# hrz2000/CustomNeRF

Hardware: AMD Instinct MI355X
Metric: training rays/s (higher is better)
Workload: dtype f16

## Files before the change

customnerf_amd/csrc/gridencoder_binned.hip:

```cpp
#include "grid_common.h"
#include "optim_common.h"
#include <vector>
#include <algorithm>
#include <cstdio>

#define BN_CHUNK_LOG2 12
#define BN_CHUNK (1u << BN_CHUNK_LOG2)
#define BN_THREADS 256
#define BN_PPT 4
#define BN_PTS (BN_THREADS * BN_PPT)
#define BN_MAX_CHUNKS 512
#define BN_SEG (1u << 18)

struct BinPlan {
    uint32_t bin_first[GE_MAX_LEVELS + 1];
    uint32_t nb;
    uint32_t total_bins;
};

struct BinWs {
    uint32_t *hist;
    uint32_t *bin_base;
    uint32_t *seg_first;
    void *records;
// ... 123 lines not shown
        }
        __syncthreads();
        if (tid == 0) { carry_r = cr + tr; carry_s = cs + ts; }
        __syncthreads();
    }
    if (tid == 0) {
        bin_base[total_bins] = carry_r; seg_first[total_bins] = carry_s;
        if (split_list) split_list[0] = n_split;
    }
}

template <typename T>
__global__ void __launch_bounds__(BN_THREADS) k_bin_emit(const T *__restrict__ grad, const float *__restrict__ inputs, const GridLevels lv,
                                                         const BinPlan plan, const uint32_t *__restrict__ hist,
                                                         const uint32_t *__restrict__ bin_base, BinRec<T> *__restrict__ records, uint32_t B,
                                                         uint32_t gridtype, int align_corners, uint32_t interp, float *__restrict__ grad_grid,
                                                         float *__restrict__ found_inf) {
    __shared__ uint32_t cursor[BN_MAX_CHUNKS];
    const uint32_t level = blockIdx.x / plan.nb, pb = blockIdx.x % plan.nb;
    const uint32_t nch = plan.bin_first[level + 1] - plan.bin_first[level];
    for (uint32_t c = threadIdx.x; c < nch; c += BN_THREADS) {
        const uint32_t bin = plan.bin_first[level] + c;
        cursor[c] = bin_base[bin] + hist[(size_t)bin * plan.nb + pb];
    }
    __syncthreads();
#pragma unroll
    for (int i = 0; i < BN_PPT; i++) {
        const uint32_t b = pb * BN_PTS + i * BN_THREADS + threadIdx.x;
        float in[3];
        if (!bn_load_point(inputs, b, B, in)) continue;
        uint32_t index[8];
        float wgt[8];
        bn_corners(in, lv, level, gridtype, align_corners, interp, index, wgt);
        using Vec = FeatVec<T, 2>;
        const Vec g = reinterpret_cast<const Vec *>(grad)[(size_t)level * B + b];
        const float g0 = ge_to_float(g.v[0]), g1 = ge_to_float(g.v[1]);
        if constexpr (sizeof(T) == 2) {
            if (!(fabsf(g0) <= 65504.0f) || !(fabsf(g1) <= 65504.0f)) {
                grad_grid[((size_t)lv.offset[level] + index[0]) * 2] = __builtin_nanf("");
                if (found_inf) *found_inf = 1.0f;
            }
        } else {
            if ((!(fabsf(g0) <= 3.4e38f) || !(fabsf(g1) <= 3.4e38f)) && found_inf) *found_inf = 1.0f;
        }
        struct alignas(8) RecPair { BinRec<T> a, b; };
#pragma unroll
        for (int q = 0; q < 4; q++) {
            const uint32_t i0 = index[2 * q], i1 = index[2 * q + 1];
            const uint32_t c0 = i0 >> BN_CHUNK_LOG2, c1 = i1 >> BN_CHUNK_LOG2;
            RecPair rp;
            rp.a.idx = i0 & (BN_CHUNK - 1);
            rp.b.idx = i1 & (BN_CHUNK - 1);
            if constexpr (sizeof(T) == 2) {
                rp.a.v = __floats2half2_rn(wgt[2 * q] * g0, wgt[2 * q] * g1);
                rp.b.v = __floats2half2_rn(wgt[2 * q + 1] * g0, wgt[2 * q + 1] * g1);
            } else {
                rp.a.v0 = wgt[2 * q] * g0; rp.a.v1 = wgt[2 * q] * g1;
                rp.b.v0 = wgt[2 * q + 1] * g0; rp.b.v1 = wgt[2 * q + 1] * g1;
            }
            const uint32_t pos0 = atomicAdd(&cursor[c0], c0 == c1 ? 2u : 1u);
            if (c0 == c1) {
                *reinterpret_cast<RecPair *>(records + pos0) = rp;
            } else {
                const uint32_t pos1 = atomicAdd(&cursor[c1], 1u);
                records[pos0] = rp.a;
                records[pos1] = rp.b;
            }
        }
    }
}

#define BN_FIX_BITS 24
template <typename T> struct BinAcc;
template <> struct BinAcc<__half> { using type = long long; };
template <> struct BinAcc<float> { using type = float; };

template <typename T>
__device__ __forceinline__ void bn_add_record(typename BinAcc<T>::type *acc, const BinRec<T> &r) {
    if constexpr (sizeof(T) == 2) {
        const float2 f = __half22float2(r.v);
        const long long a = (long long)(f.x * 16777216.0f), b = (long long)(f.y * 16777216.0f);
        atomicAdd(reinterpret_cast<unsigned long long *>(&acc[r.idx * 2]), (unsigned long long)a);
        atomicAdd(reinterpret_cast<unsigned long long *>(&acc[r.idx * 2 + 1]), (unsigned long long)b);
    } else {
        unsafeAtomicAdd(&acc[r.idx * 2], r.v0);
        unsafeAtomicAdd(&acc[r.idx * 2 + 1], r.v1);
    }
}

template <typename T>
__device__ __forceinline__ float bn_acc_to_float(typename BinAcc<T>::type a) {
    if constexpr (sizeof(T) == 2) return (float)((double)a * (1.0 / 16777216.0));
    else return a;
}

template <typename T>
__global__ void __launch_bounds__(1024) k_bin_accum(const BinRec<T> *__restrict__ records, const uint32_t *__restrict__ bin_base,
                                                    const uint32_t *__restrict__ seg_first, const GridLevels lv, const BinPlan plan,
                                                    float *__restrict__ grad_grid) {
    using A = typename BinAcc<T>::type;
    extern __shared__ __attribute__((aligned(16))) unsigned char bn_lds[];
    A *acc = reinterpret_cast<A *>(bn_lds);
    uint32_t &s_bin = *reinterpret_cast<uint32_t *>(bn_lds + sizeof(A) * BN_CHUNK * 2);
    const uint32_t nseg_total = seg_first[plan.total_bins];
    if (blockIdx.x >= nseg_total) return;
    if (threadIdx.x == 0) {
        uint32_t lo = 0, hi = plan.total_bins;
        while (lo < hi) {
            const uint32_t mid = (lo + hi) >> 1;
            if (seg_first[mid + 1] <= blockIdx.x) lo = mid + 1; else hi = mid;
        }
        s_bin = lo;
    }
    for (uint32_t i = threadIdx.x; i < sizeof(A) * BN_CHUNK * 2 / 16; i += 1024) reinterpret_cast<uint4 *>(bn_lds)[i] = make_uint4(0, 0, 0, 0);
    __syncthreads();
    const uint32_t bin = s_bin;
    const uint32_t seg = blockIdx.x - seg_first[bin], nseg = seg_first[bin + 1] - seg_first[bin];
    const uint32_t r0 = bin_base[bin], r1 = bin_base[bin + 1];
    const uint32_t begin = r0 + seg * BN_SEG, end = min(begin + BN_SEG, r1);
    constexpr int UNR = 4;
    uint32_t i = begin + threadIdx.x;
    for (; i + (UNR - 1) * 1024 < end; i += UNR * 1024) {
        BinRec<T> r[UNR];
#pragma unroll
        for (int u = 0; u < UNR; u++) r[u] = records[i + u * 1024];
#pragma unroll
        for (int u = 0; u < UNR; u++) bn_add_record<T>(acc, r[u]);
    }
    for (; i < end; i += 1024) bn_add_record<T>(acc, records[i]);
    __syncthreads();
    uint32_t level = 0;
    while (plan.bin_first[level + 1] <= bin) level++;
    const uint32_t chunk = bin - plan.bin_first[level];
    const uint32_t e0 = chunk << BN_CHUNK_LOG2;
    const uint32_t n_entries = min(BN_CHUNK, lv.size[level] - e0);
    float *__restrict__ dst = grad_grid + ((size_t)lv.offset[level] + e0) * 2;
    if (nseg == 1) {
        for (uint32_t j = threadIdx.x; j < n_entries * 2 / 4; j += 1024) {
            float4 g = reinterpret_cast<float4 *>(dst)[j];
            g.x += bn_acc_to_float<T>(acc[j * 4]); g.y += bn_acc_to_float<T>(acc[j * 4 + 1]);
            g.z += bn_acc_to_float<T>(acc[j * 4 + 2]); g.w += bn_acc_to_float<T>(acc[j * 4 + 3]);
            reinterpret_cast<float4 *>(dst)[j] = g;
        }
    } else {
        for (uint32_t j = threadIdx.x; j < n_entries * 2; j += 1024) {
            const float a = bn_acc_to_float<T>(acc[j]);
            if (a != 0.0f) unsafeAtomicAdd(&dst[j], a);
        }
    }
}


#define B3_SINGLE 15u


__device__ __forceinline__ void b3_pairs(const float (&in)[3], const GridLevels &lv, uint32_t level, uint32_t gridtype, bool align_corners,
                                         uint32_t interp, uint32_t (&i0)[4], uint32_t (&i1)[4], float (&wyz)[4], float &fx) {
    const uint32_t hashmap_size = lv.size[level];
    const float scale = lv.scale[level];
    const uint32_t resolution = lv.resolution[level];
    float pos[3];
    uint32_t pos_grid[3];
#pragma unroll
    for (int d = 0; d < 3; d++) {
        pos[d] = cn_fma(in[d], scale, align_corners ? 0.0f : 0.5f);
        pos_grid[d] = (uint32_t)floorf(pos[d]);
        pos[d] -= (float)pos_grid[d];
        if (interp == 1) pos[d] = ge_smoothstep(pos[d]);
    }
    fx = pos[0];
    const float oy = 1 - pos[1], oz = 1 - pos[2];
    wyz[0] = oy * oz; wyz[1] = pos[1] * oz; wyz[2] = oy * pos[2]; wyz[3] = pos[1] * pos[2];
    const int mode = ge_level_mode<3>(gridtype, align_corners, hashmap_size, resolution);
    if (mode == GE_MODE_HASH2) {
        const uint32_t mask = hashmap_size - 1;
        const uint32_t hy0 = pos_grid[1] * 2654435761u, hy1 = hy0 + 2654435761u, hz0 = pos_grid[2] * 805459861u, hz1 = hz0 + 805459861u;
        const uint32_t hyz[4] = {hy0 ^ hz0, hy1 ^ hz0, hy0 ^ hz1, hy1 ^ hz1};
        const uint32_t x0 = pos_grid[0], x1 = x0 + 1;
#pragma unroll
        for (int q = 0; q < 4; q++) { i0[q] = (x0 ^ hyz[q]) & mask; i1[q] = (x1 ^ hyz[q]) & mask; }
    } else if (mode == GE_MODE_DENSE) {
        const uint32_t s1 = align_corners ? resolution : resolution + 1, s2 = s1 * s1;
        const uint32_t lin = pos_grid[0] + pos_grid[1] * s1 + pos_grid[2] * s2;
        i0[0] = lin; i0[1] = lin + s1; i0[2] = lin + s2; i0[3] = lin + s1 + s2;
#pragma unroll
        for (int q = 0; q < 4; q++) i1[q] = i0[q] + 1;
        if (align_corners) {
#pragma unroll
            for (int q = 0; q < 4; q++) {
                if (i0[q] >= hashmap_size) i0[q] -= hashmap_size;
                if (i1[q] >= hashmap_size) i1[q] -= hashmap_size;
            }
        }
    } else {
        ge_dispatch_mode(mode, [&](auto mode_c) {
#pragma unroll
        for (int q = 0; q < 4; q++) {
            uint32_t pgl[3] = {pos_grid[0], pos_grid[1] + (q & 1), pos_grid[2] + (q >> 1)};
            i0[q] = ge_index_m<3, decltype(mode_c)::value>(gridtype, align_corners, hashmap_size, resolution, pgl);
            pgl[0] += 1;
            i1[q] = ge_index_m<3, decltype(mode_c)::value>(gridtype, align_corners, hashmap_size, resolution, pgl);
        }
        });
    }
}

__device__ __forceinline__ bool b3_paired_d(uint32_t i0, uint32_t i1) {
    const uint32_t m = i0 ^ i1;
    return m != 0 && (m >> BN_CHUNK_LOG2) == 0 && (m & (m + 1)) == 0;
}

__device__ __forceinline__ uint32_t b3_ticket(uint32_t *counters, uint32_t c) {
    const uint64_t act = __ballot(1);
    const uint32_t c_lead = __builtin_amdgcn_readfirstlane(c);
    if (__ballot(c == c_lead) == act) {
        const uint32_t rank = __builtin_amdgcn_mbcnt_hi((uint32_t)(act >> 32), __builtin_amdgcn_mbcnt_lo((uint32_t)act, 0u));
        uint32_t base = 0;
        if (rank == 0) base = atomicAdd(&counters[c_lead], (uint32_t)__popcll(act));
        return __builtin_amdgcn_readfirstlane(base) + rank;
    }
    return atomicAdd(&counters[c], 1u);
}

__device__ __forceinline__ void b3_poison(float g0, float g1, float *__restrict__ grad_grid, const GridLevels &lv, uint32_t level, uint32_t entry,
                                          float *__restrict__ found_inf) {
    if (!(fabsf(g0) <= 65504.0f) || !(fabsf(g1) <= 65504.0f)) {
        grad_grid[((size_t)lv.offset[level] + entry) * 2] = __builtin_nanf("");
        if (found_inf) *found_inf = 1.0f;
    }
}

__device__ __forceinline__ unsigned long long b3_fix(float a) {
    const double y = (double)a + 6755399441055744.0;
    return __builtin_bit_cast(unsigned long long, y) - 0x4338000000000000ull;
}
__device__ __forceinline__ void b3_add(long long *acc, uint32_t e, float a, float b) {
    atomicAdd(reinterpret_cast<unsigned long long *>(&acc[e]), b3_fix(a));
    atomicAdd(reinterpret_cast<unsigned long long *>(&acc[BN_CHUNK + e]), b3_fix(b));
}

__device__ __forceinline__ void b3_add_record(long long *acc, const uint2 r) {
    union { uint32_t u; __half2 h; } v;
    v.u = r.y;
    const float2 f = __half22float2(v.h);
    const uint32_t e = r.x & (BN_CHUNK - 1), t = (r.x >> 12) & 15u;
    if (t == B3_SINGLE) {
        b3_add(acc, e, f.x * 16777216.0f, f.y * 16777216.0f);
    } else {
        const float w1 = (float)(r.x >> 16) * (1.0f / 65536.0f), w0 = 1.0f - w1;
        const float w1s = w1 * 16777216.0f, w0s = w0 * 16777216.0f;
        b3_add(acc, e, w0s * f.x, w0s * f.y);
        b3_add(acc, e ^ ((2u << t) - 1u), w1s * f.x, w1s * f.y);
    }
}

#ifndef B3_WALK
#define B3_WALK 8
#endif
struct B3Pending { uint32_t key; unsigned long long a0, b0, a1, b1; };
__device__ __forceinline__ void b3_flush_pending(long long *acc, const B3Pending &c) {
    if (c.key == 0xFFFFFFFFu) return;
    const uint32_t e = c.key & (BN_CHUNK - 1), t = (c.key >> 12) & 15u;
    atomicAdd(reinterpret_cast<unsigned long long *>(&acc[e]), c.a0);
    atomicAdd(reinterpret_cast<unsigned long long *>(&acc[BN_CHUNK + e]), c.b0);
    if (t != B3_SINGLE) {
        const uint32_t e1 = e ^ ((2u << t) - 1u);
        atomicAdd(reinterpret_cast<unsigned long long *>(&acc[e1]), c.a1);
        atomicAdd(reinterpret_cast<unsigned long long *>(&acc[BN_CHUNK + e1]), c.b1);
    }
}
__device__ __forceinline__ void b3_push_record(long long *acc, B3Pending &c, const uint2 r) {
    union { uint32_t u; __half2 h; } v;
    v.u = r.y;
    const float2 f = __half22float2(v.h);
    const uint32_t key = r.x & 0xFFFFu, t = (r.x >> 12) & 15u;
    unsigned long long a0, b0, a1 = 0, b1 = 0;
    if (t == B3_SINGLE) {
        a0 = b3_fix(f.x * 16777216.0f); b0 = b3_fix(f.y * 16777216.0f);
    } else {
        const float w1 = (float)(r.x >> 16) * (1.0f / 65536.0f), w0 = 1.0f - w1;
        const float w1s = w1 * 16777216.0f, w0s = w0 * 16777216.0f;
        a0 = b3_fix(w0s * f.x); b0 = b3_fix(w0s * f.y);
        a1 = b3_fix(w1s * f.x); b1 = b3_fix(w1s * f.y);
    }
    if (key == c.key) {
        c.a0 += a0; c.b0 += b0; c.a1 += a1; c.b1 += b1;
    } else {
        b3_flush_pending(acc, c);
        c.key = key; c.a0 = a0; c.b0 = b0; c.a1 = a1; c.b1 = b1;
    }
}

#ifndef B3_PTS
#define B3_PTS 2048
#endif
#ifndef B3_THREADS
#define B3_THREADS 1024
#endif
#define B3_CAP (B3_PTS * 4 + 640)
#define B3_NARROW_CHUNKS 128
#define B3_WIDE_CHUNKS BN_MAX_CHUNKS
#ifndef B3_WALK_BLOCKS
#define B3_WALK_BLOCKS 256
#endif
#define B3_MAXT (B3_WALK_BLOCKS + 8)
#define B3_REGION (B3_PTS * 8)

struct Bin3Slots {
    uint32_t bin_first[GE_MAX_LEVELS + 1];
    uint32_t nb;
    uint32_t total_bins;
};

struct Bin3Plan {
    Bin3Slots p;
    uint32_t capb;
    uint32_t dense_slot[GE_MAX_LEVELS];
    uint8_t hbits[GE_MAX_LEVELS];
};

#ifndef B3_K
#define B3_K 7u
#endif
__device__ __forceinline__ uint32_t b3_bin_of(uint32_t e, uint32_t hbits) { return (e >> B3_K) & ((1u << hbits) - 1u); }
__device__ __forceinline__ uint32_t b3_local_of(uint32_t e, uint32_t hbits) { return ((e >> (B3_K + hbits)) << B3_K) | (e & ((1u << B3_K) - 1u)); }
__device__ __forceinline__ uint32_t b3_entry_of(uint32_t local, uint32_t bin, uint32_t hbits) {
    return ((local >> B3_K) << (B3_K + hbits)) | (bin << B3_K) | (local & ((1u << B3_K) - 1u));
}
__device__ __forceinline__ bool b3_paired_h(uint32_t i0, uint32_t i1) {
    const uint32_t m = i0 ^ i1;
    return m != 0 && m < (1u << B3_K) && (m & (m + 1)) == 0;
}

__global__ void __launch_bounds__(B3_THREADS, B3_THREADS >= 1024 ? 8 : 4) k_bin3_emit(const __half *__restrict__ grad, const float *__restrict__ inputs, const GridLevels lv,
                                                          const Bin3Plan plan, uint32_t *__restrict__ runs, uint32_t *__restrict__ cursor,
                                                          uint2 *__restrict__ hslab, uint2 *__restrict__ dslab, uint32_t B,
                                                          uint32_t gridtype, int align_corners, uint32_t interp, float *__restrict__ grad_grid, uint32_t n_slots,
                                                          uint32_t abl_arg, float *__restrict__ found_inf) {
#ifdef CNERF_TUNING
    const uint32_t abl = abl_arg;
#else
    constexpr uint32_t abl = 0;
    (void)abl_arg;
#endif
    extern __shared__ __attribute__((aligned(16))) unsigned char b3_lds[];
    uint2 *s_rec = reinterpret_cast<uint2 *>(b3_lds);
    uint8_t *s_bin = b3_lds + (size_t)B3_CAP * 8;
    const uint32_t nb = plan.p.nb;
    const uint32_t slot = blockIdx.x % n_slots, pb = blockIdx.x / n_slots;
    const uint32_t level = lv.order[slot];
    const uint32_t bin0 = plan.p.bin_first[slot], nch = plan.p.bin_first[slot + 1] - bin0;
    const bool dense_lvl = plan.dense_slot[slot] != 0xFFFFFFFFu;
    const uint32_t hb = plan.hbits[slot];
    const bool wide = nch > B3_NARROW_CHUNKS;
    const uint32_t NBN = wide ? B3_WIDE_CHUNKS : B3_NARROW_CHUNKS;
    uint32_t *cnt = reinterpret_cast<uint32_t *>(b3_lds + (size_t)B3_CAP * (wide ? 8 : 9));
    uint32_t *start = cnt + NBN;
    uint32_t *gdst = start + NBN;
    uint32_t *s_total = gdst + NBN;
    auto bin_of = [&](uint32_t e) { return dense_lvl ? e >> BN_CHUNK_LOG2 : b3_bin_of(e, hb); };
    auto local_of = [&](uint32_t e) { return dense_lvl ? e & (BN_CHUNK - 1) : b3_local_of(e, hb); };
    auto paired = [&](uint32_t a, uint32_t b) { return dense_lvl ? b3_paired_d(a, b) : b3_paired_h(a, b); };
    if (threadIdx.x < NBN) cnt[threadIdx.x] = 0;
    __syncthreads();
    constexpr int PPT = B3_PTS / B3_THREADS;
    bool ok[PPT];
    uint32_t i0[PPT][4], i1[PPT][4], tk[PPT][4];
    float wyz[PPT][4], fx[PPT], g0[PPT], g1[PPT];
    float in_[PPT][3];
    FeatVec<__half, 2> gh[PPT];
#pragma unroll
    for (int i = 0; i < PPT; i++) {
        const uint32_t bc = min(pb * B3_PTS + i * B3_THREADS + threadIdx.x, B - 1);
        ge_load_coords<3>(inputs, bc, in_[i]);
        gh[i] = reinterpret_cast<const FeatVec<__half, 2> *>(grad)[(size_t)level * B + bc];
    }
#pragma unroll
    for (int i = 0; i < PPT; i++) {
        const uint32_t b = pb * B3_PTS + i * B3_THREADS + threadIdx.x;
        const float (&in)[3] = in_[i];
        ok[i] = b < B && !(in[0] < 0 || in[0] > 1 || in[1] < 0 || in[1] > 1 || in[2] < 0 || in[2] > 1);
        g0[i] = __half2float(gh[i].v[0]); g1[i] = __half2float(gh[i].v[1]);
        ok[i] = ok[i] && (g0[i] != 0.0f || g1[i] != 0.0f);
        fx[i] = 0.0f;
        if (ok[i]) {
            if (abl & 32) {
#pragma unroll
                for (int q = 0; q < 4; q++) { i0[i][q] = (b * 4 + q) * 2654435761u % lv.size[level]; i1[i][q] = i0[i][q] ^ 1u; wyz[i][q] = 0.25f; }
                fx[i] = in[0] - floorf(in[0]);
            } else {
                b3_pairs(in, lv, level, gridtype, align_corners, interp, i0[i], i1[i], wyz[i], fx[i]);
            }
            b3_poison(g0[i], g1[i], grad_grid, lv, level, i0[i][0], found_inf);
#pragma unroll
            for (int q = 0; q < 4; q++) {
                if (abl & 16) { tk[i][q] = 0; continue; }
                const uint32_t c0 = bin_of(i0[i][q]);
                if (paired(i0[i][q], i1[i][q])) {
                    tk[i][q] = dense_lvl ? b3_ticket(cnt, c0) : atomicAdd(&cnt[c0], 1u);
                } else {
                    const uint32_t t0 = atomicAdd(&cnt[c0], 1u);
                    const uint32_t t1 = atomicAdd(&cnt[bin_of(i1[i][q])], 1u);
                    tk[i][q] = t0 | (t1 << 16);
                }
            }
        }
    }
    __syncthreads();
    uint32_t res_a = 0, res_b = 0;
    if (wide) {
        if (threadIdx.x < 64) {
            const uint32_t lane = threadIdx.x;
            constexpr uint32_t KPL = B3_WIDE_CHUNKS / 64;
            uint32_t c8[KPL], loc = 0;
#pragma unroll
            for (uint32_t k = 0; k < KPL; k++) { c8[k] = cnt[lane * KPL + k]; loc += c8[k]; }
            const uint32_t incl = cn_wave_incl_scan(loc);
            uint32_t run = incl - loc;
#pragma unroll
            for (uint32_t k = 0; k < KPL; k++) {
                const uint32_t c = lane * KPL + k;
                start[c] = run;
                if (dense_lvl && c < nch && !(abl & 8)) runs[(size_t)(bin0 + c) * nb + pb] = c8[k] | (run << 16);
                run += c8[k];
            }
            if (lane == 63) *s_total = incl;
        }
        asm volatile("s_waitcnt lgkmcnt(0)" ::: "memory");
        __builtin_amdgcn_s_barrier();
        asm volatile("" ::: "memory");
        if (!dense_lvl && !(abl & 1) && threadIdx.x <= NBN / 2) {
            const uint32_t b_lo = ((bin0 >> 1) + threadIdx.x) * 2u;
            uint32_t sa[2] = {0u, 0u};
#pragma unroll
            for (int h = 0; h < 2; h++) {
                const uint32_t c = b_lo + h - bin0;
                if (c < nch) {
                    const uint32_t n = cnt[c], st0 = start[c];
                    sa[h] = st0 >= B3_CAP ? 0u : min(n, (uint32_t)B3_CAP - st0);
                }
            }
            if (sa[0] | sa[1]) {
                const unsigned long long old = atomicAdd(reinterpret_cast<unsigned long long *>(cursor + b_lo), (unsigned long long)sa[0] | ((unsigned long long)sa[1] << 32));
                res_a = (uint32_t)old & 0x7FFFFFFFu;
                res_b = (uint32_t)(old >> 32) & 0x7FFFFFFFu;
            }
        }
    } else if (threadIdx.x < 64) {
        const uint32_t lane = threadIdx.x;
        const uint32_t ca = cnt[2 * lane], cb = cnt[2 * lane + 1];
        const uint32_t incl = cn_wave_incl_scan(ca + cb);
        const uint32_t oa = incl - (ca + cb), ob = oa + ca;
        start[2 * lane] = oa; start[2 * lane + 1] = ob;
        if (lane == 63) *s_total = incl;
        if (dense_lvl) {
            if (2 * lane < nch && !(abl & 8)) runs[(size_t)(bin0 + 2 * lane) * nb + pb] = ca | (oa << 16);
            if (2 * lane + 1 < nch && !(abl & 8)) runs[(size_t)(bin0 + 2 * lane + 1) * nb + pb] = cb | (ob << 16);
        } else if (!(abl & 1)) {
            const uint32_t sa = (2 * lane < nch && oa < B3_CAP) ? min(ca, (uint32_t)B3_CAP - oa) : 0u;
            const uint32_t sb = (2 * lane + 1 < nch && ob < B3_CAP) ? min(cb, (uint32_t)B3_CAP - ob) : 0u;
            if ((bin0 & 1u) == 0) {
                if (sa | sb) {
                    const unsigned long long old = atomicAdd(reinterpret_cast<unsigned long long *>(cursor + bin0 + 2 * lane),
                                                             (unsigned long long)sa | ((unsigned long long)sb << 32));
                    res_a = (uint32_t)old & 0x7FFFFFFFu;
                    res_b = (uint32_t)(old >> 32) & 0x7FFFFFFFu;
                }
            } else {
                if (sa) res_a = atomicAdd(&cursor[bin0 + 2 * lane], sa) & 0x7FFFFFFFu;
                if (sb) res_b = atomicAdd(&cursor[bin0 + 2 * lane + 1], sb) & 0x7FFFFFFFu;
            }
        }
    }
    asm volatile("s_waitcnt lgkmcnt(0)" ::: "memory");
    __builtin_amdgcn_s_barrier();
    asm volatile("" ::: "memory");
    uint2 *__restrict__ region = dslab + ((size_t)slot * nb + pb) * B3_REGION;
#pragma unroll
    for (int i = 0; i < PPT; i++) {
        if (!ok[i] || (abl & 4)) continue;
        const uint32_t fxq = min((uint32_t)(fx[i] * 65536.0f), 65535u);
        union { __half2 h; uint32_t u; } v;
        auto put = [&](uint32_t c, uint32_t ticket, uint32_t word, uint32_t val) {
            const uint32_t sl = start[c] + ticket;
            if (sl < B3_CAP) { s_rec[sl] = make_uint2(word, val); if (!wide) s_bin[sl] = (uint8_t)c; }
            else region[sl] = make_uint2(word, val);
        };
#pragma unroll
        for (int q = 0; q < 4; q++) {
            const uint32_t a0 = i0[i][q], a1 = i1[i][q];
            const uint32_t c0 = bin_of(a0);
            if (paired(a0, a1)) {
                const uint32_t t = 31u - (uint32_t)__clz((int)(a0 ^ a1));
                v.h = __floats2half2_rn(wyz[i][q] * g0[i], wyz[i][q] * g1[i]);
                put(c0, tk[i][q], local_of(a0) | (t << 12) | (fxq << 16), v.u);
            } else {
                const float w0 = (1 - fx[i]) * wyz[i][q], w1 = fx[i] * wyz[i][q];
                v.h = __floats2half2_rn(w0 * g0[i], w0 * g1[i]);
                put(c0, tk[i][q] & 0xFFFFu, local_of(a0) | (B3_SINGLE << 12), v.u);
                v.h = __floats2half2_rn(w1 * g0[i], w1 * g1[i]);
                put(bin_of(a1), tk[i][q] >> 16, local_of(a1) | (B3_SINGLE << 12), v.u);
            }
        }
    }
    if (!dense_lvl && wide) {
        if (threadIdx.x <= NBN / 2) {
            const uint32_t capb = plan.capb, b_lo = ((bin0 >> 1) + threadIdx.x) * 2u;
#pragma unroll
            for (int h = 0; h < 2; h++) {
                const uint32_t c = b_lo + h - bin0;
                if (c >= nch) continue;
                const uint32_t n = cnt[c], st0 = start[c], res = h ? res_b : res_a;
                const uint32_t staged = st0 >= B3_CAP ? 0u : min(n, (uint32_t)B3_CAP - st0);
                const uint32_t room = res >= capb ? 0u : capb - res;
                const uint32_t fit = min(min(n, room), staged);
                gdst[c] = res - st0;
                cnt[c] = fit;
                if (!(abl & 8)) runs[(size_t)(bin0 + c) * nb + pb] = (n - fit) | ((st0 + fit) << 16);
                if (n > fit) atomicOr(&cursor[bin0 + c], 0x80000000u);
            }
        }
    } else if (!dense_lvl && threadIdx.x < 64) {
        const uint32_t capb = plan.capb;
#pragma unroll
        for (int h = 0; h < 2; h++) {
            const uint32_t c = 2 * threadIdx.x + h;
            const uint32_t n = cnt[c], st0 = start[c], res = h ? res_b : res_a;
            const uint32_t staged = st0 >= B3_CAP ? 0u : min(n, (uint32_t)B3_CAP - st0);
            const uint32_t room = res >= capb ? 0u : capb - res;
            const uint32_t fit = min(min(n, room), staged);
            gdst[c] = res - st0;
            cnt[c] = fit;
            if (c < nch && !(abl & 8)) runs[(size_t)(bin0 + c) * nb + pb] = (n - fit) | ((st0 + fit) << 16);
            if (c < nch && n > fit) atomicOr(&cursor[bin0 + c], 0x80000000u);
        }
    }
    __syncthreads();
    const uint32_t total = (abl & 2) ? 0u : min(*s_total, (uint32_t)B3_CAP);
    if (dense_lvl) {
        for (uint32_t sl = threadIdx.x; sl < total; sl += B3_THREADS) region[sl] = s_rec[sl];
    } else if (wide) {
        const uint32_t capb = plan.capb, l16 = threadIdx.x & 15, grp = threadIdx.x >> 4;
        for (uint32_t c = grp; c < nch; c += B3_THREADS / 16) {
            const uint32_t st0 = start[c], en = min(c + 1 < NBN ? start[c + 1] : *s_total, total), fit = cnt[c], gd = gdst[c];
            for (uint32_t sl = st0 + l16; sl < en; sl += 16) {
                if (sl - st0 < fit) hslab[(size_t)(bin0 + c) * capb + (gd + sl)] = s_rec[sl];
                else region[sl] = s_rec[sl];
            }
        }
    } else {
        const uint32_t capb = plan.capb;
        for (uint32_t sl = threadIdx.x; sl < total; sl += B3_THREADS) {
            const uint32_t c = s_bin[sl];
            const uint32_t pos = gdst[c] + sl;
            if (sl - start[c] < cnt[c]) hslab[(size_t)(bin0 + c) * capb + pos] = s_rec[sl];
            else region[sl] = s_rec[sl];
        }
    }
}

__global__ void __launch_bounds__(BN_SCAN_THREADS) k_bin3_totals(const uint32_t *__restrict__ runs, uint32_t *__restrict__ pre, const uint32_t *__restrict__ cursor,
                                                                 uint32_t *__restrict__ bin_total, const Bin3Plan plan, uint32_t n_slots) {
    constexpr uint32_t NW = BN_SCAN_THREADS / 64;
    __shared__ uint32_t wave_tot[NW];
    __shared__ uint32_t carry;
    const uint32_t bin = blockIdx.x, nb = plan.p.nb;
    uint32_t slot = 0;
    while (slot + 1 < n_slots && plan.p.bin_first[slot + 1] <= bin) slot++;
    const bool hashed = plan.dense_slot[slot] == 0xFFFFFFFFu;
    if (hashed) {
        const uint32_t cw = cursor[bin], c = cw & 0x7FFFFFFFu;
        if (!(cw >> 31)) {
            if (threadIdx.x == 0) bin_total[bin] = min(c, plan.capb);
            return;
        }
    }
    const uint32_t *h = runs + (size_t)bin * nb;
    uint32_t *o = pre + (size_t)bin * nb;
    const uint32_t tid = threadIdx.x, lane = tid & 63, wave = tid >> 6;
    if (tid == 0) carry = 0;
    __syncthreads();
    for (uint32_t s0 = 0; s0 < nb; s0 += BN_SCAN_THREADS * 4) {
        const uint32_t i = s0 + tid * 4;
        uint32_t v[4];
#pragma unroll
        for (int k = 0; k < 4; k++) v[k] = i + k < nb ? (h[i + k] & 0xFFFFu) : 0;
        const uint32_t mine = v[0] + v[1] + v[2] + v[3];
        const uint32_t incl = cn_wave_incl_scan(mine);
        if (lane == 63) wave_tot[wave] = incl;
        __syncthreads();
        uint32_t wbase = 0, tot = 0;
#pragma unroll
        for (uint32_t w = 0; w < NW; w++) {
            const uint32_t t = wave_tot[w];
            if (w < wave) wbase += t;
            tot += t;
        }
        const uint32_t base = carry;
        uint32_t run = base + wbase + incl - mine;
#pragma unroll
        for (int k = 0; k < 4; k++) {
            if (i + k < nb) o[i + k] = run;
            run += v[k];
        }
        __syncthreads();
        if (tid == 0) carry = base + tot;
        __syncthreads();
    }
    if (tid == 0) bin_total[bin] = hashed ? min(cursor[bin] & 0x7FFFFFFFu, plan.capb) + carry : carry;
}

struct B3Adam {
    float *p, *m, *v;
    __half *ph;
    const float *state;
    float lr, beta1, beta2, eps, extra_inv;
    int zero_grad, on;
    const float *cst;
};
struct B3AdamConst { float gscale, step_size, rsqrt_bc2; int skip; };
__device__ __forceinline__ B3AdamConst b3_adam_const(const B3Adam &ad) {
    B3AdamConst c;
    c.gscale = ad.cst[0]; c.step_size = ad.cst[1]; c.rsqrt_bc2 = ad.cst[2]; c.skip = ad.cst[3] != 0.0f;
    return c;
}
__device__ __forceinline__ void b3_adam_update(const B3Adam &ad, const B3AdamConst &c, size_t idx, float4 gg, float4 pp, float4 mm, float4 vv, float4 *d4) {
    const CnAdamK ak = {c.gscale, c.step_size, c.rsqrt_bc2, ad.beta1, ad.beta2, ad.eps};
    float *pa = &pp.x, *ga = &gg.x, *ma = &mm.x, *va = &vv.x;
#pragma unroll
    for (int k = 0; k < 4; k++) cn_adam_elem(pa[k], ma[k], va[k], ga[k], ak);
    *reinterpret_cast<float4 *>(ad.p + idx) = pp;
    *reinterpret_cast<float4 *>(ad.m + idx) = mm;
    *reinterpret_cast<float4 *>(ad.v + idx) = vv;
    *d4 = ad.zero_grad ? make_float4(0, 0, 0, 0) : gg;
    if (ad.ph) *reinterpret_cast<uint2 *>(ad.ph + idx) = cn_pack_half4(pp);
}
__device__ __forceinline__ void b3_adam_apply(const B3Adam &ad, const B3AdamConst &c, size_t idx, float4 gg, float4 *d4) {
    if (c.skip) {
        *d4 = ad.zero_grad ? make_float4(0, 0, 0, 0) : gg;
        return;
    }
    b3_adam_update(ad, c, idx, gg, *reinterpret_cast<const float4 *>(ad.p + idx), *reinterpret_cast<const float4 *>(ad.m + idx),
                   *reinterpret_cast<const float4 *>(ad.v + idx), d4);
}

__device__ __forceinline__ void b3_flush(const long long *acc, const GridLevels &lv, const Bin3Slots &plan, uint32_t slot, uint32_t bin, uint32_t nseg, uint32_t gseg,
                                         float *__restrict__ grad_grid, long long *__restrict__ partial, uint32_t hbits, const B3Adam &ad,
                                         const B3AdamConst &adc) {
    const uint32_t level = lv.order[slot];
    const uint32_t cb = bin - plan.bin_first[slot];
    const uint32_t e0 = hbits == 0xFFu ? cb << BN_CHUNK_LOG2 : 0u;
    const uint32_t n_entries = hbits == 0xFFu ? min(BN_CHUNK, lv.size[level] - e0) : min(BN_CHUNK, lv.size[level] >> hbits);
    float *__restrict__ dst = grad_grid + (size_t)lv.offset[level] * 2;
    if (nseg == 1 && ad.on && !adc.skip) {
        constexpr int NIT = BN_CHUNK / 2 / 1024;
        float4 gg[NIT], pp[NIT], mm[NIT], vv[NIT];
        auto index_of = [&](uint32_t j) {
            const uint32_t e = hbits == 0xFFu ? e0 + 2 * j : b3_entry_of(2 * j, cb, hbits);
            return ((size_t)lv.offset[level] + e) * 2;
        };
#pragma unroll
        for (int it = 0; it < NIT; it++) {
            const uint32_t j = it * 1024 + threadIdx.x;
            if (j < n_entries / 2) {
                const size_t idx = index_of(j);
                gg[it] = *reinterpret_cast<const float4 *>(grad_grid + idx);
                pp[it] = *reinterpret_cast<const float4 *>(ad.p + idx);
                mm[it] = *reinterpret_cast<const float4 *>(ad.m + idx);
                vv[it] = *reinterpret_cast<const float4 *>(ad.v + idx);
            }
        }
#pragma unroll
        for (int it = 0; it < NIT; it++) {
            const uint32_t j = it * 1024 + threadIdx.x;
            if (j >= n_entries / 2) continue;
            const size_t idx = index_of(j);
            float4 g = gg[it];
            g.x += bn_acc_to_float<__half>(acc[j * 2]); g.y += bn_acc_to_float<__half>(acc[BN_CHUNK + j * 2]);
            g.z += bn_acc_to_float<__half>(acc[j * 2 + 1]); g.w += bn_acc_to_float<__half>(acc[BN_CHUNK + j * 2 + 1]);
            b3_adam_update(ad, adc, idx, g, pp[it], mm[it], vv[it], reinterpret_cast<float4 *>(grad_grid + idx));
        }
    } else if (nseg == 1) {
        for (uint32_t j = threadIdx.x; j < n_entries / 2; j += 1024) {
            const uint32_t e = hbits == 0xFFu ? e0 + 2 * j : b3_entry_of(2 * j, cb, hbits);
            float4 *d4 = reinterpret_cast<float4 *>(dst + (size_t)e * 2);
            float4 g = *d4;
            g.x += bn_acc_to_float<__half>(acc[j * 2]); g.y += bn_acc_to_float<__half>(acc[BN_CHUNK + j * 2]);
            g.z += bn_acc_to_float<__half>(acc[j * 2 + 1]); g.w += bn_acc_to_float<__half>(acc[BN_CHUNK + j * 2 + 1]);
            if (ad.on) b3_adam_apply(ad, adc, ((size_t)lv.offset[level] + e) * 2, g, d4);
            else *d4 = g;
        }
    } else {
        long long *__restrict__ img = partial + (size_t)gseg * (BN_CHUNK * 2);
        for (uint32_t j = threadIdx.x; j < n_entries * 2; j += 1024) img[j] = acc[(j & 1) * BN_CHUNK + (j >> 1)];
    }
}

#define B3_RS_GROUPS 64
#ifndef B3_RS_BINS
#define B3_RS_BINS 256
#endif
__global__ void __launch_bounds__(256) k_bin3_reduce_split(const long long *__restrict__ partial, const uint32_t *__restrict__ seg_first,
                                                           const GridLevels lv, const Bin3Plan plan, float *__restrict__ grad_grid, uint32_t n_slots,
                                                           const uint32_t *__restrict__ split_list, const B3Adam ad) {
    __shared__ long long s_sum[3][B3_RS_GROUPS][4];
    const uint32_t n_split = split_list ? split_list[0] : gridDim.x;
    if (blockIdx.x >= n_split) return;
    B3AdamConst adc = {0.0f, 0.0f, 0.0f, 0};
    if (ad.on) adc = b3_adam_const(ad);
    for (uint32_t b = blockIdx.x; b < n_split; b += gridDim.x) {
    const uint32_t bin = split_list ? split_list[1 + b] : b;
// ... 247 lines not shown
    return (uint32_t)((s + k - 1) / k);
}

static uint32_t b3_max_bins(const Bin3Slots &plan, uint32_t nl) {
    uint32_t m = 1;
    for (uint32_t s = 0; s < nl; s++) m = m > plan.bin_first[s + 1] - plan.bin_first[s] ? m : plan.bin_first[s + 1] - plan.bin_first[s];
    return m;
}

struct Bin3Ws {
    uint32_t *runs, *pre, *cursor, *bin_base, *seg_first, *seg_bin, *split_list;
    float *adam_const;
    uint2 *hslab, *dslab;
    long long *partial;
    uint64_t max_seg, cursor_bytes;
};

static bool b3_is_dense(const GridLevels &lv, uint32_t level, int ac) {
    const uint64_t r1 = (uint64_t)lv.resolution[level] + (ac ? 0 : 1);
    return r1 * r1 * r1 <= lv.size[level];
}

static bool b3_plan(const GridLevels &lv, uint32_t nl, uint32_t B, Bin3Plan &plan, uint32_t &n_dense, int ac) {
    Bin3Slots &ps = plan.p;
    ps.nb = cn_div_up(B, B3_PTS);
    uint32_t acc = 0;
    for (uint32_t s = 0; s < nl; s++) {
        ps.bin_first[s] = acc;
        acc += cn_div_up(lv.size[lv.order[s]], BN_CHUNK);
    }
    for (uint32_t s = nl; s <= GE_MAX_LEVELS; s++) ps.bin_first[s] = acc;
    ps.total_bins = acc;
    n_dense = 0;
    uint64_t cap = 0;
    bool ok = true;
    for (uint32_t s = 0; s < GE_MAX_LEVELS; s++) { plan.dense_slot[s] = 0xFFFFFFFFu; plan.hbits[s] = 0; }
    for (uint32_t s = 0; s < nl; s++) {
        const uint32_t level = lv.order[s], size = lv.size[level];
        if (b3_is_dense(lv, level, ac)) { plan.dense_slot[s] = n_dense++; continue; }
        const uint32_t nch = ps.bin_first[s + 1] - ps.bin_first[s];
        if ((size & (size - 1)) != 0 || (nch & (nch - 1)) != 0 || !(size == nch * BN_CHUNK || (nch == 1 && size >= 32))) ok = false;
        uint32_t hb = 0;
        while ((1u << hb) < nch) hb++;
        plan.hbits[s] = (uint8_t)hb;
        const uint64_t mean = (uint64_t)B * 17 / 4 / nch;
        const uint64_t c = mean + mean / 2 + 8192;
        cap = cap > c ? cap : c;
    }
    plan.capb = (uint32_t)((cap + 1) & ~(uint64_t)1);
    return ok;
}

static bool b3_enabled(const GridLevels &lv, uint32_t nl, uint32_t B, int dtype, uint32_t gridtype, int ac) {
    static const int on = cn_tune_env("CNERF_B3", 1);
    static const int wide_on = cn_tune_env("CNERF_B3_WIDE", 1);
    (void)gridtype;
    if (!on || dtype != CNERF_F16) return false;
    Bin3Plan plan;
    uint32_t nd;
    if (!b3_plan(lv, nl, B, plan, nd, ac)) return false;
    const uint32_t mc = b3_max_bins(plan.p, nl);
    if (mc > (wide_on ? (uint32_t)B3_WIDE_CHUNKS : (uint32_t)B3_NARROW_CHUNKS)) return false;
    if ((uint64_t)plan.p.total_bins * plan.capb >= 0xF0000000ull) return false;
    return (uint64_t)nl * plan.p.nb * B3_REGION < 0xF0000000ull && (uint64_t)B * 8 < 0x7FFFFFFFull;
}

static uint64_t b3_layout(const Bin3Plan &plan, uint32_t n_dense, uint32_t B, uint32_t nl, Bin3Ws *ws, void *base) {
    const Bin3Slots &ps = plan.p;
    uint64_t off = 0;
    const uint64_t o_runs = off; off = bn_align(off + (uint64_t)ps.total_bins * ps.nb * 4);
    const uint64_t o_pre = off; off = bn_align(off + (uint64_t)ps.total_bins * ps.nb * 4);
    const uint64_t o_cur = off; off = bn_align(off + ((uint64_t)ps.total_bins + 2) * 4);
    const uint64_t o_base = off; off = bn_align(off + (uint64_t)(ps.total_bins + 1) * 4);
    const uint64_t o_seg = off; off = bn_align(off + (uint64_t)(ps.total_bins + 1) * 4);
    const uint64_t o_split = off; off = bn_align(off + (uint64_t)(ps.total_bins + 1) * 4);
    const uint64_t o_adamc = off; off = bn_align(off + 16);
    const uint64_t h_records = (uint64_t)ps.total_bins * plan.capb;
    const uint64_t d_records = (uint64_t)nl * ps.nb * B3_REGION;
    (void)n_dense;
    const uint64_t o_h = off; off = bn_align(off + h_records * 8);
    const uint64_t o_d = off; off = bn_align(off + d_records * 8);
    const uint64_t max_seg = (uint64_t)ps.total_bins + cn_div_up64((uint64_t)B * nl * 8, b3_seg(B, b3_max_bins(ps, nl)));
    const uint64_t o_segbin = off; off = bn_align(off + max_seg * 4);
    const uint64_t o_part = off; off = bn_align(off + max_seg * BN_CHUNK * 2 * 8);
    if (ws) {
        char *p = (char *)base;
        ws->runs = (uint32_t *)(p + o_runs);
        ws->pre = (uint32_t *)(p + o_pre);
        ws->cursor = (uint32_t *)(p + o_cur);
        ws->cursor_bytes = (uint64_t)ps.total_bins * 4;
        ws->bin_base = (uint32_t *)(p + o_base);
        ws->seg_first = (uint32_t *)(p + o_seg);
        ws->split_list = (uint32_t *)(p + o_split);
        ws->adam_const = (float *)(p + o_adamc);
        ws->hslab = (uint2 *)(p + o_h);
        ws->dslab = (uint2 *)(p + o_d);
        ws->seg_bin = (uint32_t *)(p + o_segbin);
        ws->partial = (long long *)(p + o_part);
        ws->max_seg = max_seg;
    }
    return off;
}

__global__ void __launch_bounds__(256) k_bin3_zero(uint32_t *__restrict__ p, uint32_t n) {
    const uint32_t i = blockIdx.x * 256 + threadIdx.x;
    if (i < n) p[i] = 0;
}

static CnerfGridAdam g_grid_adam;
static bool g_grid_adam_armed = false;
static int g_grid_adam_consumed = 0;
void bn_grid_adam_arm(const CnerfGridAdam *cfg) {
    g_grid_adam_armed = cfg != nullptr;
    if (cfg) { g_grid_adam = *cfg; g_grid_adam_consumed = 0; }
}
int bn_grid_adam_consumed() { const int c = g_grid_adam_consumed; g_grid_adam_consumed = 0; return c; }
static B3Adam b3_take_adam(float *gemb, const GridLevels &lv, uint32_t nl, bool third_form) {
    B3Adam ad = {};
    if (!g_grid_adam_armed || g_grid_adam.g != gemb) return ad;
    g_grid_adam_armed = false;
    const uint64_t covered = ((uint64_t)lv.offset[nl - 1] + lv.size[nl - 1]) * 2;
    if (!third_form || covered != g_grid_adam.n) return ad;
    ad.p = g_grid_adam.p; ad.m = g_grid_adam.m; ad.v = g_grid_adam.v; ad.ph = reinterpret_cast<__half *>(g_grid_adam.p_half);
    ad.state = g_grid_adam.scaler_state;
    ad.lr = g_grid_adam.lr; ad.beta1 = g_grid_adam.beta1; ad.beta2 = g_grid_adam.beta2; ad.eps = g_grid_adam.eps; ad.extra_inv = g_grid_adam.extra_inv;
    ad.zero_grad = g_grid_adam.zero_grad; ad.on = 1;
    g_grid_adam_consumed = 1;
    return ad;
}

static int b3_backward(const __half *grad, const float *inputs, const GridLevels &lv, float *gemb, uint32_t B, uint32_t nl, uint32_t gridtype, int ac,
                       uint32_t interp, void *workspace, hipStream_t st) {
    if (nl == 0) return CNERF_OK;
    Bin3Plan plan;
    uint32_t n_dense;
    if (!b3_plan(lv, nl, B, plan, n_dense, ac)) return CNERF_EINVAL;
    Bin3Ws ws;
    b3_layout(plan, n_dense, B, nl, &ws, workspace);
    static const int emit_pad = cn_tune_env("CNERF_B3_EMIT_LDS_PAD", 0);
    const uint32_t lds_n = B3_CAP * 9 + B3_NARROW_CHUNKS * 12 + 16, lds_w = B3_CAP * 8 + B3_WIDE_CHUNKS * 12 + 16;
    const uint32_t emit_lds = (lds_n > lds_w ? lds_n : lds_w) + (uint32_t)emit_pad, acc_lds = BN_CHUNK * 2 * sizeof(long long) + 32 + B3_MAXT * 8;
    static bool attr_set = false;
    if (!attr_set) {
        (void)hipFuncSetAttribute(reinterpret_cast<const void *>(&k_bin3_emit), hipFuncAttributeMaxDynamicSharedMemorySize, emit_lds);
        (void)hipFuncSetAttribute(reinterpret_cast<const void *>(&k_bin3_accum), hipFuncAttributeMaxDynamicSharedMemorySize, acc_lds);
        attr_set = true;
    }
    const Bin3Slots &ps = plan.p;
    const uint32_t seg = b3_seg(B, b3_max_bins(ps, nl));
    B3Adam ad = b3_take_adam(gemb, lv, nl, true);
    ad.cst = ws.adam_const;
    hipLaunchKernelGGL(k_bin3_zero, dim3(cn_div_up(ps.total_bins, 256)), dim3(256), 0, st, ws.cursor, ps.total_bins);
    cn_stage(0, st);
    hipLaunchKernelGGL(k_bin3_emit, dim3(ps.nb * nl), dim3(B3_THREADS), emit_lds, st, grad, inputs, lv, plan, ws.runs, ws.cursor, ws.hslab, ws.dslab, B, gridtype, ac,
                       interp, gemb, nl, (uint32_t)cn_tune_env("CNERF_B3_EMIT_ABL", 0), g_cn_found_inf);
    cn_stage(1, st);
    hipLaunchKernelGGL(k_bin3_totals, dim3(ps.total_bins), dim3(BN_SCAN_THREADS), 0, st, (const uint32_t *)ws.runs, ws.pre, (const uint32_t *)ws.cursor, ws.bin_base,
                       plan, nl);
    static const uint32_t rs_bins = (uint32_t)cn_tune_env("CNERF_B3_RS_BINS", B3_RS_BINS);
    static const int rs_list = cn_tune_env("CNERF_B3_RSLIST", 1);
    hipLaunchKernelGGL(k_bin_scan_bins, dim3(1), dim3(1024), 0, st, ws.bin_base, ws.bin_base, ws.seg_first, ps.total_bins, seg, ws.seg_bin, ws.split_list, ad.on,
                       ad.state, ad.lr, ad.beta1, ad.beta2, ad.extra_inv, ad.on ? ws.adam_const : (float *)nullptr);
    hipLaunchKernelGGL(k_bin3_accum, dim3((uint32_t)ws.max_seg), dim3(1024), acc_lds, st, (const uint2 *)ws.hslab, (const uint2 *)ws.dslab, (const uint32_t *)ws.runs,
                       (const uint32_t *)ws.pre, (const uint32_t *)ws.cursor, (const uint32_t *)ws.bin_base, (const uint32_t *)ws.seg_first, lv, plan, gemb, ws.partial,
                       (const uint32_t *)ws.seg_bin, nl, seg, (uint32_t)cn_tune_env("CNERF_B3_ONLY", 0), ad);
    cn_stage(2, st);
    hipLaunchKernelGGL(k_bin3_reduce_split, dim3(!rs_list || ps.total_bins < rs_bins ? ps.total_bins : rs_bins, BN_CHUNK * 2 / 4 / B3_RS_GROUPS), dim3(256), 0, st,
                       (const long long *)ws.partial, ws.seg_first, lv, plan, gemb, nl, rs_list ? (const uint32_t *)ws.split_list : (const uint32_t *)nullptr, ad);
    cn_stage(3, st);
#ifdef CNERF_TUNING
    static const int dbg = cn_tune_env("CNERF_B3_DEBUG", 0);
    static int dbg_calls = 0;
    if (dbg && (++dbg_calls % dbg) == 0) {
        uint32_t n_split = 0, n_seg = 0;
        (void)hipStreamSynchronize(st);
        (void)hipMemcpy(&n_split, ws.split_list, 4, hipMemcpyDeviceToHost);
        (void)hipMemcpy(&n_seg, ws.seg_first + ps.total_bins, 4, hipMemcpyDeviceToHost);
        std::vector<uint32_t> sf(ps.total_bins + 1), bb(ps.total_bins + 1);
        (void)hipMemcpy(sf.data(), ws.seg_first, sf.size() * 4, hipMemcpyDeviceToHost);
        (void)hipMemcpy(bb.data(), ws.bin_base, bb.size() * 4, hipMemcpyDeviceToHost);
        fprintf(stderr, "[b3] call %d: bins %u segments %u split bins %u seg %u | per slot (bins, segments, records, max bin):", dbg_calls, ps.total_bins, n_seg, n_split, seg);
        for (uint32_t sl = 0; sl < nl; sl++) {
            uint32_t mx = 0;
            for (uint32_t b_ = ps.bin_first[sl]; b_ < ps.bin_first[sl + 1]; b_++) mx = std::max(mx, bb[b_ + 1] - bb[b_]);
            fprintf(stderr, " L%u(%u,%u,%u,%u)", lv.order[sl], ps.bin_first[sl + 1] - ps.bin_first[sl], sf[ps.bin_first[sl + 1]] - sf[ps.bin_first[sl]],
                    bb[ps.bin_first[sl + 1]] - bb[ps.bin_first[sl]], mx);
        }
        fprintf(stderr, "\n");
    }
#endif
    return cn_launch_status();
}

bool bn_eligible(uint32_t B, uint32_t D, uint32_t C, uint32_t nl, const GridLevels &lv) {
    if (D != 3 || C != 2 || nl == 0) return false;
    for (uint32_t l = 0; l < nl; l++)
        if (cn_div_up(lv.size[l], BN_CHUNK) > BN_MAX_CHUNKS || (lv.size[l] & 7)) return false;
    return (uint64_t)B * nl * 8 < 0xF0000000ull;
}

uint64_t bn_workspace_bytes(uint32_t B, uint32_t nl, const GridLevels &lv, int dtype) {
    uint64_t b3 = 0;
    for (int ac = 0; ac < 2; ac++) {
        if (!b3_enabled(lv, nl, B, dtype, 0u, ac)) continue;
        Bin3Plan p3;
        uint32_t nd;
        b3_plan(lv, nl, B, p3, nd, ac);
        const uint64_t b = b3_layout(p3, nd, B, nl, nullptr, nullptr);
        b3 = b > b3 ? b : b3;
    }
    BinPlan plan;
    bn_plan(lv, nl, B, plan);
    const uint64_t b1 = bn_layout(plan, B, nl, dtype, nullptr, nullptr);
    return b1 > b3 ? b1 : b3;
}

static int bn_prepare(const float *inputs, const GridLevels &lv, uint32_t B, uint32_t nl, uint32_t gridtype, int ac, uint32_t interp, int dtype,
               void *workspace, hipStream_t st) {
    BinPlan plan;
    bn_plan(lv, nl, B, plan);
    BinWs ws;
    bn_layout(plan, B, nl, dtype, &ws, workspace);
    const dim3 grid1(plan.nb * nl);
    hipLaunchKernelGGL(k_bin_hist, grid1, dim3(BN_THREADS), 0, st, inputs, lv, plan, ws.hist, B, gridtype, ac, interp);
    hipLaunchKernelGGL(k_bin_scan_blocks, dim3(plan.total_bins), dim3(BN_SCAN_THREADS), 0, st, ws.hist, ws.bin_base, plan.nb);
    hipLaunchKernelGGL(k_bin_scan_bins, dim3(1), dim3(1024), 0, st, ws.bin_base, ws.bin_base, ws.seg_first, plan.total_bins, BN_SEG, (uint32_t *)nullptr);
    return cn_launch_status();
}

template <typename T>
static int bn_phase2(const T *grad, const float *inputs, const GridLevels &lv, float *gemb, uint32_t B, uint32_t nl, uint32_t gridtype, int ac,
                     uint32_t interp, int dtype, void *workspace, hipStream_t st) {
    BinPlan plan;
    bn_plan(lv, nl, B, plan);
    BinWs ws;
    bn_layout(plan, B, nl, dtype, &ws, workspace);
    const dim3 grid1(plan.nb * nl);
    hipLaunchKernelGGL((k_bin_emit<T>), grid1, dim3(BN_THREADS), 0, st, grad, inputs, lv, plan, ws.hist, ws.bin_base, (BinRec<T> *)ws.records, B,
                       gridtype, ac, interp, gemb, g_cn_found_inf);
    const uint64_t max_seg = (uint64_t)plan.total_bins + cn_div_up64((uint64_t)B * nl * 8, BN_SEG);
    const uint32_t lds_bytes = BN_CHUNK * 2 * sizeof(typename BinAcc<T>::type) + 16;
    static bool attr_set = false;
    if (!attr_set) {
        (void)hipFuncSetAttribute(reinterpret_cast<const void *>(&k_bin_accum<T>), hipFuncAttributeMaxDynamicSharedMemorySize, lds_bytes);
        attr_set = true;
    }
    hipLaunchKernelGGL((k_bin_accum<T>), dim3((uint32_t)max_seg), dim3(1024), lds_bytes, st, (const BinRec<T> *)ws.records,
                       ws.bin_base, ws.seg_first, lv, plan, gemb);
    return cn_launch_status();
}

int bn_backward(const void *grad, const float *inputs, const GridLevels &lv, float *gemb, uint32_t B, uint32_t nl, uint32_t gridtype, int ac,
                uint32_t interp, int dtype, void *workspace, hipStream_t st) {
    if (b3_enabled(lv, nl, B, dtype, gridtype, ac)) return b3_backward((const __half *)grad, inputs, lv, gemb, B, nl, gridtype, ac, interp, workspace, st);
    if (nl) (void)b3_take_adam(gemb, lv, nl, false);
    const int rc = bn_prepare(inputs, lv, B, nl, gridtype, ac, interp, dtype, workspace, st);
    if (rc) return rc;
    if (dtype == CNERF_F16) return bn_phase2<__half>((const __half *)grad, inputs, lv, gemb, B, nl, gridtype, ac, interp, dtype, workspace, st);
    return bn_phase2<float>((const float *)grad, inputs, lv, gemb, B, nl, gridtype, ac, interp, dtype, workspace, st);
}
```

Measured before the change: 8.617 million.

## Use single ticket per point when all corners fall in one dense bin

The emit kernel is split into a templated body, and a dispatcher picks a two-class variant for dense levels with few chunks. In that variant, a point whose eight corners all land in the same bin takes one LDS atomic ticket instead of four. Its four records go into a separate per-bin sub-region that the scan sizes as four times the ticket count. This cuts shared-memory atomic traffic in the binning pass, at the cost of more code paths, a changed scan layout and register pressure from template duplication. Tuning-only ablation hooks are also added.

```diff
diff --git a/customnerf_amd/csrc/gridencoder_binned.hip b/customnerf_amd/csrc/gridencoder_binned.hip
--- a/customnerf_amd/csrc/gridencoder_binned.hip
+++ b/customnerf_amd/csrc/gridencoder_binned.hip
@@ -299,6 +299,8 @@
 
 
 #define B3_SINGLE 15u
+#define B3_ABL_CELL 14u
+#define B3_ABL_TAIL 13u
 
 
 __device__ __forceinline__ void b3_pairs(const float (&in)[3], const GridLevels &lv, uint32_t level, uint32_t gridtype, bool align_corners,
@@ -368,6 +370,19 @@
     }
     return atomicAdd(&counters[c], 1u);
 }
+#ifdef CNERF_TUNING
+__device__ __forceinline__ uint32_t b3_ticket_n(uint32_t *counters, uint32_t c, uint32_t n) {
+    const uint64_t act = __ballot(1);
+    const uint32_t c_lead = __builtin_amdgcn_readfirstlane(c);
+    if (__ballot(c == c_lead) == act) {
+        const uint32_t rank = __builtin_amdgcn_mbcnt_hi((uint32_t)(act >> 32), __builtin_amdgcn_mbcnt_lo((uint32_t)act, 0u));
+        uint32_t base = 0;
+        if (rank == 0) base = atomicAdd(&counters[c_lead], (uint32_t)__popcll(act) * n);
+        return __builtin_amdgcn_readfirstlane(base) + rank * n;
+    }
+    return atomicAdd(&counters[c], n);
+}
+#endif
 
 __device__ __forceinline__ void b3_poison(float g0, float g1, float *__restrict__ grad_grid, const GridLevels &lv, uint32_t level, uint32_t entry,
                                           float *__restrict__ found_inf) {
@@ -408,6 +423,19 @@
 __device__ __forceinline__ void b3_flush_pending(long long *acc, const B3Pending &c) {
     if (c.key == 0xFFFFFFFFu) return;
     const uint32_t e = c.key & (BN_CHUNK - 1), t = (c.key >> 12) & 15u;
+#ifdef CNERF_TUNING
+    if (t == B3_ABL_CELL) {
+#pragma unroll
+        for (uint32_t k = 0; k < 4; k++) {
+            const uint32_t ek = (e + (k & 1u) * 289u + (k >> 1) * 17u) & (BN_CHUNK - 1), ek1 = ek ^ 1u;
+            atomicAdd(reinterpret_cast<unsigned long long *>(&acc[ek]), c.a0);
+            atomicAdd(reinterpret_cast<unsigned long long *>(&acc[BN_CHUNK + ek]), c.b0);
+            atomicAdd(reinterpret_cast<unsigned long long *>(&acc[ek1]), c.a1);
+            atomicAdd(reinterpret_cast<unsigned long long *>(&acc[BN_CHUNK + ek1]), c.b1);
+        }
+        return;
+    }
+#endif
     atomicAdd(reinterpret_cast<unsigned long long *>(&acc[e]), c.a0);
     atomicAdd(reinterpret_cast<unsigned long long *>(&acc[BN_CHUNK + e]), c.b0);
     if (t != B3_SINGLE) {
@@ -421,6 +449,9 @@
     v.u = r.y;
     const float2 f = __half22float2(v.h);
     const uint32_t key = r.x & 0xFFFFu, t = (r.x >> 12) & 15u;
+#ifdef CNERF_TUNING
+    if (t == B3_ABL_TAIL) return;
+#endif
     unsigned long long a0, b0, a1 = 0, b1 = 0;
     if (t == B3_SINGLE) {
         a0 = b3_fix(f.x * 16777216.0f); b0 = b3_fix(f.y * 16777216.0f);
@@ -479,13 +510,15 @@
     return m != 0 && m < (1u << B3_K) && (m & (m + 1)) == 0;
 }
 
-__global__ void __launch_bounds__(B3_THREADS, B3_THREADS >= 1024 ? 8 : 4) k_bin3_emit(const __half *__restrict__ grad, const float *__restrict__ inputs, const GridLevels lv,
+template <bool TWO>
+__device__ __forceinline__ void b3_emit(const __half *__restrict__ grad, const float *__restrict__ inputs, const GridLevels lv,
                                                           const Bin3Plan plan, uint32_t *__restrict__ runs, uint32_t *__restrict__ cursor,
                                                           uint2 *__restrict__ hslab, uint2 *__restrict__ dslab, uint32_t B,
                                                           uint32_t gridtype, int align_corners, uint32_t interp, float *__restrict__ grad_grid, uint32_t n_slots,
                                                           uint32_t abl_arg, float *__restrict__ found_inf) {
 #ifdef CNERF_TUNING
     const uint32_t abl = abl_arg;
+    bool cell[B3_PTS / B3_THREADS];
 #else
     constexpr uint32_t abl = 0;
     (void)abl_arg;
@@ -508,11 +541,14 @@
     auto bin_of = [&](uint32_t e) { return dense_lvl ? e >> BN_CHUNK_LOG2 : b3_bin_of(e, hb); };
     auto local_of = [&](uint32_t e) { return dense_lvl ? e & (BN_CHUNK - 1) : b3_local_of(e, hb); };
     auto paired = [&](uint32_t a, uint32_t b) { return dense_lvl ? b3_paired_d(a, b) : b3_paired_h(a, b); };
+    constexpr bool two_class = TWO;
+    if (TWO) __builtin_assume(dense_lvl && nch <= B3_NARROW_CHUNKS / 2);
     if (threadIdx.x < NBN) cnt[threadIdx.x] = 0;
     __syncthreads();
     constexpr int PPT = B3_PTS / B3_THREADS;
     bool ok[PPT];
     uint32_t i0[PPT][4], i1[PPT][4], tk[PPT][4];
+    auto one_ticket = [&](int i) { return two_class && !(abl & (16u | 32u | 384u)) && i1[i][3] > i0[i][0] && bin_of(i1[i][3]) == bin_of(i0[i][0]); };
     float wyz[PPT][4], fx[PPT], g0[PPT], g1[PPT];
     float in_[PPT][3];
     FeatVec<__half, 2> gh[PPT];
@@ -539,6 +575,17 @@
                 b3_pairs(in, lv, level, gridtype, align_corners, interp, i0[i], i1[i], wyz[i], fx[i]);
             }
             b3_poison(g0[i], g1[i], grad_grid, lv, level, i0[i][0], found_inf);
+#ifdef CNERF_TUNING
+            cell[i] = (abl & 384u) && dense_lvl && nch <= 64 && i1[i][3] > i0[i][0] && bin_of(i1[i][3]) == bin_of(i0[i][0]);
+            if (cell[i]) {
+                tk[i][0] = (abl & 16) ? 0u : b3_ticket_n(cnt, bin_of(i0[i][0]), (abl & 256u) ? 2u : 1u);
+                continue;
+            }
+#endif
+            if (one_ticket(i)) {
+                tk[i][0] = b3_ticket(cnt, B3_NARROW_CHUNKS / 2 + bin_of(i0[i][0]));
+                continue;
+            }
 #pragma unroll
             for (int q = 0; q < 4; q++) {
                 if (abl & 16) { tk[i][q] = 0; continue; }
@@ -595,10 +642,21 @@
         }
     } else if (threadIdx.x < 64) {
         const uint32_t lane = threadIdx.x;
-        const uint32_t ca = cnt[2 * lane], cb = cnt[2 * lane + 1];
-        const uint32_t incl = cn_wave_incl_scan(ca + cb);
-        const uint32_t oa = incl - (ca + cb), ob = oa + ca;
-        start[2 * lane] = oa; start[2 * lane + 1] = ob;
+        uint32_t ca = cnt[2 * lane], cb = cnt[2 * lane + 1], sa = 0, sb = 0;
+        if (two_class) {
+            constexpr uint32_t H = B3_NARROW_CHUNKS / 2;
+            if (lane < H / 2) { sa = 4u * cnt[H + 2 * lane]; sb = 4u * cnt[H + 2 * lane + 1]; }
+            else ca = cb = 0;
+        }
+        const uint32_t incl = cn_wave_incl_scan(sa + ca + sb + cb);
+        const uint32_t oa = incl - (sa + ca + sb + cb), ob = oa + sa + ca;
+        if (two_class) {
+            constexpr uint32_t H = B3_NARROW_CHUNKS / 2;
+            if (lane < H / 2) { start[H + 2 * lane] = oa; start[2 * lane] = oa + sa; start[H + 2 * lane + 1] = ob; start[2 * lane + 1] = ob + sb; }
+        } else {
+            start[2 * lane] = oa; start[2 * lane + 1] = ob;
+        }
+        ca += sa; cb += sb;
         if (lane == 63) *s_total = incl;
         if (dense_lvl) {
             if (2 * lane < nch && !(abl & 8)) runs[(size_t)(bin0 + 2 * lane) * nb + pb] = ca | (oa << 16);
@@ -633,6 +691,24 @@
             if (sl < B3_CAP) { s_rec[sl] = make_uint2(word, val); if (!wide) s_bin[sl] = (uint8_t)c; }
             else region[sl] = make_uint2(word, val);
         };
+#ifdef CNERF_TUNING
+        if (cell[i]) {
+            v.h = __floats2half2_rn(wyz[i][0] * g0[i], wyz[i][0] * g1[i]);
+            put(bin_of(i0[i][0]), tk[i][0], local_of(i0[i][0]) | (B3_ABL_CELL << 12) | (fxq << 16), v.u);
+            if (abl & 256u) put(bin_of(i0[i][0]), tk[i][0] + 1, local_of(i0[i][0]) | (B3_ABL_TAIL << 12) | (fxq << 16), v.u);
+            continue;
+        }
+#endif
+        if (one_ticket(i)) {
+            const uint32_t c = B3_NARROW_CHUNKS / 2 + bin_of(i0[i][0]), n = cnt[c];
+#pragma unroll
+            for (int q = 0; q < 4; q++) {
+                const uint32_t t = 31u - (uint32_t)__clz((int)(i0[i][q] ^ i1[i][q]));
+                v.h = __floats2half2_rn(wyz[i][q] * g0[i], wyz[i][q] * g1[i]);
+                put(c, tk[i][0] + (uint32_t)q * n, local_of(i0[i][q]) | (t << 12) | (fxq << 16), v.u);
+            }
+            continue;
+        }
 #pragma unroll
         for (int q = 0; q < 4; q++) {
             const uint32_t a0 = i0[i][q], a1 = i1[i][q];
@@ -704,6 +780,18 @@
             else region[sl] = s_rec[sl];
         }
     }
+}
+
+__global__ void __launch_bounds__(B3_THREADS, B3_THREADS >= 1024 ? 8 : 4) k_bin3_emit(const __half *__restrict__ grad, const float *__restrict__ inputs, const GridLevels lv,
+                                                          const Bin3Plan plan, uint32_t *__restrict__ runs, uint32_t *__restrict__ cursor,
+                                                          uint2 *__restrict__ hslab, uint2 *__restrict__ dslab, uint32_t B,
+                                                          uint32_t gridtype, int align_corners, uint32_t interp, float *__restrict__ grad_grid, uint32_t n_slots,
+                                                          uint32_t abl_arg, float *__restrict__ found_inf) {
+    const uint32_t slot = blockIdx.x % n_slots;
+    if (plan.dense_slot[slot] != 0xFFFFFFFFu && plan.p.bin_first[slot + 1] - plan.p.bin_first[slot] <= B3_NARROW_CHUNKS / 2)
+        b3_emit<true>(grad, inputs, lv, plan, runs, cursor, hslab, dslab, B, gridtype, align_corners, interp, grad_grid, n_slots, abl_arg, found_inf);
+    else
+        b3_emit<false>(grad, inputs, lv, plan, runs, cursor, hslab, dslab, B, gridtype, align_corners, interp, grad_grid, n_slots, abl_arg, found_inf);
 }
 
 __global__ void __launch_bounds__(BN_SCAN_THREADS) k_bin3_totals(const uint32_t *__restrict__ runs, uint32_t *__restrict__ pre, const uint32_t *__restrict__ cursor,
@@ -1257,8 +1345,13 @@
     ad.cst = ws.adam_const;
     hipLaunchKernelGGL(k_bin3_zero, dim3(cn_div_up(ps.total_bins, 256)), dim3(256), 0, st, ws.cursor, ps.total_bins);
     cn_stage(0, st);
+    uint32_t emit_abl = (uint32_t)cn_tune_env("CNERF_B3_EMIT_ABL", 0);
+#ifdef CNERF_TUNING
+    static int abl_calls = 0;
+    if (abl_calls++ < cn_tune_env("CNERF_B3_EMIT_ABL_AFTER", 0)) emit_abl = 0;
+#endif
     hipLaunchKernelGGL(k_bin3_emit, dim3(ps.nb * nl), dim3(B3_THREADS), emit_lds, st, grad, inputs, lv, plan, ws.runs, ws.cursor, ws.hslab, ws.dslab, B, gridtype, ac,
-                       interp, gemb, nl, (uint32_t)cn_tune_env("CNERF_B3_EMIT_ABL", 0), g_cn_found_inf);
+                       interp, gemb, nl, emit_abl, g_cn_found_inf);
     cn_stage(1, st);
     hipLaunchKernelGGL(k_bin3_totals, dim3(ps.total_bins), dim3(BN_SCAN_THREADS), 0, st, (const uint32_t *)ws.runs, ws.pre, (const uint32_t *)ws.cursor, ws.bin_base,
                        plan, nl);
```

After: 8.768 million, median of 6. +1.8%, better.
